# google-research/Splat-SLAM

Hardware: AMD Instinct MI355X
Metric: mapping frames/sec + render ms @640x480, 300k Gaussians; PSNR vs ref (higher is better)
Workload: dtype f32

## Files before the change

splat_slam_amd/csrc/sgr_aux.hip:

```cpp
#include <cmath>

#include <cstdint>

#include "sgr_common.h"

namespace sgr {
int set_error(int code, const char* fmt, ...);


__global__ void __launch_bounds__(256) mapping_loss_kernel(LossTab tab, int HW, float w_rgb, float w_dep, float thr) {
  const int vw = blockIdx.y;
  const float* __restrict__ image = tab.image[vw];
  const float* __restrict__ depth = tab.depth[vw];
  const float* __restrict__ gt_image = tab.gt_image[vw];
  const float* __restrict__ gt_depth = tab.gt_depth[vw];
  float* __restrict__ dimage = tab.dimage[vw];
  float* __restrict__ ddepth = tab.ddepth[vw];
  LossPart* __restrict__ parts = (LossPart*)tab.parts[vw];
  const float ea = tab.exp_a[vw] ? __expf(tab.exp_a[vw][0]) : 1.f;
  const float eb = tab.exp_b[vw] ? tab.exp_b[vw][0] : 0.f;
  LossPart acc = {0.f, 0.f, 0.f, 0.f};
  for (int p = blockIdx.x * blockDim.x + threadIdx.x; p < HW; p += gridDim.x * blockDim.x) {
    float g0 = gt_image[p], g1 = gt_image[HW + p], g2 = gt_image[2 * HW + p];
    bool m = (g0 + g1 + g2) > thr;
// ... 146 lines not shown
                                                       float* __restrict__ s_out, float* __restrict__ r_out,
                                                       float* __restrict__ o_out) {
#pragma clang fp contract(off)
  int64_t i = (int64_t)blockIdx.x * blockDim.x + threadIdx.x;
  if (i >= n) return;
  if (s_out) {
    const F3 sc = ld3(scaling + 3 * i);
    st3(s_out + 3 * i, F3{expf(sc.x), expf(sc.y), expf(sc.z)});
  }
  if (r_out) {
    float4 q = *(const float4*)(rotation + 4 * i);
    float nn = fmaxf(sqrtf(q.x * q.x + q.y * q.y + q.z * q.z + q.w * q.w), 1e-12f);
    *(float4*)(r_out + 4 * i) = make_float4(q.x / nn, q.y / nn, q.z / nn, q.w / nn);
  }
  if (o_out) o_out[i] = 1.f / (1.f + expf(-opacity[i]));
}

#define adam_update(p, g, m, v, GRP, c)                      \
  do {                                                       \
    m = m + (g - m) * (1.f - c.b1);                          \
    v = v * c.b2 + (1.f - c.b2) * g * g;                     \
    float denom_ = sqrtf(v) / c.bc2_sqrt[GRP] + c.eps;       \
    p = p - c.step_size[GRP] * (m / denom_);                 \
  } while (0)

template <int MODE>
__device__ __forceinline__ float take_grad(float* __restrict__ sink, int64_t j, float gathered) {
  if (MODE == 2) return gathered;
  float g = sink[j];
  sink[j] = 0.f;
  return MODE == 1 ? g + gathered : g;
}

template <int MODE>
__device__ __forceinline__ void gaussian_adam_one(int64_t i, const AdamGroups& G, const AdamConst& c, float iso_coef,
                                                  const float* e , float* __restrict__ s_out,
                                                  float* __restrict__ r_out, float* __restrict__ o_out) {
#pragma clang fp contract(off)
#pragma unroll
  for (int grp = 0; grp < 2; ++grp) {
    const SgrAdamGroup& A = G.g[grp];
    if (i < G.r0[grp] || i >= G.r1[grp]) continue;
    float g[3];
    if (MODE == 2) {
      g[0] = e[3 * grp]; g[1] = e[3 * grp + 1]; g[2] = e[3 * grp + 2];
    } else {
      F3 gs = ld3(A.grad + 3 * i);
      st3(A.grad + 3 * i, F3{0.f, 0.f, 0.f});
      g[0] = gs.x; g[1] = gs.y; g[2] = gs.z;
      if (MODE == 1) { g[0] = g[0] + e[3 * grp]; g[1] = g[1] + e[3 * grp + 1]; g[2] = g[2] + e[3 * grp + 2]; }
    }
    if (A.skip) continue;
    F3 p3 = ld3(A.param + 3 * i), m3 = ld3(A.exp_avg + 3 * i), v3 = ld3(A.exp_avg_sq + 3 * i);
    float p[3] = {p3.x, p3.y, p3.z}, m[3] = {m3.x, m3.y, m3.z}, v[3] = {v3.x, v3.y, v3.z};
#pragma unroll
    for (int k = 0; k < 3; ++k) adam_update(p[k], g[k], m[k], v[k], grp, c);
    st3(A.param + 3 * i, F3{p[0], p[1], p[2]});
    st3(A.exp_avg + 3 * i, F3{m[0], m[1], m[2]});
    st3(A.exp_avg_sq + 3 * i, F3{v[0], v[1], v[2]});
  }
  if (i >= G.r0[2] && i < G.r1[2]) {
    const SgrAdamGroup& A = G.g[2];
    float p = A.param[i];
    float sg = 1.f / (1.f + expf(-p));
    float g = take_grad<MODE>(A.grad, i, e[6]) * sg * (1.f - sg);
    if (!A.skip) {
      float m = A.exp_avg[i], v = A.exp_avg_sq[i];
      adam_update(p, g, m, v, 2, c);
      A.param[i] = p; A.exp_avg[i] = m; A.exp_avg_sq[i] = v;
    }
    if (o_out) o_out[i] = 1.f / (1.f + expf(-p));
  }
  if (i >= G.r0[3] && i < G.r1[3]) {
    const SgrAdamGroup& A = G.g[3];
    const F3 p3 = ld3(A.param + 3 * i);
    float p[3] = {p3.x, p3.y, p3.z}, s[3];
#pragma unroll
    for (int k = 0; k < 3; ++k) s[k] = expf(p[k]);
    float mean = (s[0] + s[1] + s[2]) / 3.f;
    float sg[3], ssum = 0.f;
#pragma unroll
    for (int k = 0; k < 3; ++k) { float d = s[k] - mean; sg[k] = d > 0.f ? 1.f : (d < 0.f ? -1.f : 0.f); ssum += sg[k]; }
    float gin[3];
    if (MODE == 2) {
      gin[0] = e[7]; gin[1] = e[8]; gin[2] = e[9];
    } else {
      F3 gs = ld3(A.grad + 3 * i);
      st3(A.grad + 3 * i, F3{0.f, 0.f, 0.f});
      gin[0] = gs.x; gin[1] = gs.y; gin[2] = gs.z;
      if (MODE == 1) { gin[0] = gin[0] + e[7]; gin[1] = gin[1] + e[8]; gin[2] = gin[2] + e[9]; }
    }
    if (!A.skip) {
      F3 m3 = ld3(A.exp_avg + 3 * i), v3 = ld3(A.exp_avg_sq + 3 * i);
      float m[3] = {m3.x, m3.y, m3.z}, v[3] = {v3.x, v3.y, v3.z};
#pragma unroll
      for (int k = 0; k < 3; ++k) {
        float gs = gin[k] + iso_coef * (sg[k] - ssum / 3.f);
        float g = gs * s[k];
        adam_update(p[k], g, m[k], v[k], 3, c);
      }
      st3(A.param + 3 * i, F3{p[0], p[1], p[2]});
      st3(A.exp_avg + 3 * i, F3{m[0], m[1], m[2]});
      st3(A.exp_avg_sq + 3 * i, F3{v[0], v[1], v[2]});
    }
    if (s_out) st3(s_out + 3 * i, F3{expf(p[0]), expf(p[1]), expf(p[2])});
  }
  if (i >= G.r0[4] && i < G.r1[4]) {
    const SgrAdamGroup& A = G.g[4];
    float4 x = *(const float4*)(A.param + 4 * i);
    float4 gy;
    if (MODE == 2) {
      gy = make_float4(e[10], e[11], e[12], e[13]);
    } else {
      gy = *(const float4*)(A.grad + 4 * i);
      *(float4*)(A.grad + 4 * i) = make_float4(0.f, 0.f, 0.f, 0.f);
      if (MODE == 1) { gy.x += e[10]; gy.y += e[11]; gy.z += e[12]; gy.w += e[13]; }
    }
    float nrm = sqrtf(x.x * x.x + x.y * x.y + x.z * x.z + x.w * x.w);
    float gx[4];
    if (nrm > 1e-12f) {
      float inv = 1.f / nrm;
      float y[4] = {x.x * inv, x.y * inv, x.z * inv, x.w * inv};
      float dot = y[0] * gy.x + y[1] * gy.y + y[2] * gy.z + y[3] * gy.w;
      gx[0] = (gy.x - y[0] * dot) * inv; gx[1] = (gy.y - y[1] * dot) * inv;
      gx[2] = (gy.z - y[2] * dot) * inv; gx[3] = (gy.w - y[3] * dot) * inv;
    } else {
      gx[0] = gy.x * 1e12f; gx[1] = gy.y * 1e12f; gx[2] = gy.z * 1e12f; gx[3] = gy.w * 1e12f;
    }
    float pp[4] = {x.x, x.y, x.z, x.w};
    if (!A.skip) {
      float4 m = *(const float4*)(A.exp_avg + 4 * i), v = *(const float4*)(A.exp_avg_sq + 4 * i);
      float mm[4] = {m.x, m.y, m.z, m.w}, vv[4] = {v.x, v.y, v.z, v.w};
#pragma unroll
      for (int k = 0; k < 4; ++k) adam_update(pp[k], gx[k], mm[k], vv[k], 4, c);
      *(float4*)(A.param + 4 * i) = make_float4(pp[0], pp[1], pp[2], pp[3]);
      *(float4*)(A.exp_avg + 4 * i) = make_float4(mm[0], mm[1], mm[2], mm[3]);
      *(float4*)(A.exp_avg_sq + 4 * i) = make_float4(vv[0], vv[1], vv[2], vv[3]);
    }
    if (r_out) {
      float nn = fmaxf(sqrtf(pp[0] * pp[0] + pp[1] * pp[1] + pp[2] * pp[2] + pp[3] * pp[3]), 1e-12f);
      *(float4*)(r_out + 4 * i) = make_float4(pp[0] / nn, pp[1] / nn, pp[2] / nn, pp[3] / nn);
    }
  }
}

__global__ void __launch_bounds__(256) gaussian_adam_kernel(int64_t n, AdamGroups G, AdamConst c, float iso_coef,
                                                            float* __restrict__ s_out, float* __restrict__ r_out,
                                                            float* __restrict__ o_out) {
  int64_t i = (int64_t)blockIdx.x * blockDim.x + threadIdx.x;
  if (i >= n) return;
  const float zero[14] = {0.f, 0.f, 0.f, 0.f, 0.f, 0.f, 0.f, 0.f, 0.f, 0.f, 0.f, 0.f, 0.f, 0.f};
  gaussian_adam_one<0>(i, G, c, iso_coef, zero, s_out, r_out, o_out);
}

template <int MODE>
__global__ void __launch_bounds__(256) gather_adam_kernel(ViewTab tab, int nviews, LOff L, FusedAdam fa) {
  if ((int)blockIdx.x < fa.tail_views) {
    __shared__ LossPart red[4];
    const int v = blockIdx.x;
    loss_final_view((const LossPart*)fa.tail_parts[v], fa.tail_nparts, fa.tail_inv_rgb, fa.tail_inv_dep, fa.tail_alpha,
                    fa.tail_loss[v], fa.tail_da[v], fa.tail_db[v], red);
    if (threadIdx.x == 0 && fa.exp_rows > 0 && fa.tail_da[v] && ((const SavedHeader*)tab.saved[v])->overflow == 0u) {
      const ptrdiff_t d = fa.tail_da[v] - fa.exp_grad;
      if (d >= 0 && d < (ptrdiff_t)fa.exp_rows * fa.exp_width && d % fa.exp_width == 0) {
        const int r = (int)(d / fa.exp_width);
        if (fa.exp_active[r])
          masked_adam_row(r, fa.exp_width, fa.exp_param, fa.exp_grad, fa.exp_avg, fa.exp_avg_sq, fa.exp_step, fa.exp_lr,
                          fa.exp_b1, fa.exp_b2, fa.exp_eps);
      }
    }
    return;
  }
  __shared__ const char* s_scratch[kMaxViews];
  __shared__ const int32_t* s_radii[kMaxViews];
  __shared__ uint32_t s_over[kMaxViews];
#pragma unroll
  for (int u = 0; u < kMaxViews; ++u)
    if ((int)threadIdx.x == u && u < nviews) {
      s_scratch[u] = tab.scratch[u];
      s_radii[u] = tab.radii[u];
      s_over[u] = ((const SavedHeader*)tab.saved[u])->overflow;
    }
  __syncthreads();
  uint32_t truncated = 0u;
  for (int u = 0; u < nviews; ++u) truncated |= (s_over[u] != 0u ? 1u : 0u) << u;
  const int i = ((int)blockIdx.x - fa.tail_views) * blockDim.x + threadIdx.x;
  if (i >= L.N) return;
  float a[14];
#pragma unroll
  for (int k = 0; k < 14; ++k) a[k] = 0.f;
  float st_norm = 0.f, st_cnt = 0.f, st_maxr = 0.f;
  uint32_t seen = 0u;
  for (int p = 0; p < min(L.k1_parts, nviews); ++p) seen |= ((const uint32_t*)(tab.saved[0] + L.o_vismask))[(size_t)p * L.N + i];
  seen &= ~truncated;
  const bool any = seen != 0u;
  while (seen) {
    const int v = __builtin_ctz(seen);
    seen &= seen - 1u;
    const float4* rec = (const float4*)(s_scratch[v] + L.o_gradrec) + (size_t)i * 4;
    const int r = s_radii[v][i];
    float4 r0 = rec[0], r1 = rec[1], r2 = rec[2], r3 = rec[3];
    a[0] += r0.x; a[1] += r0.y; a[2] += r0.z; a[3] += r0.w; a[4] += r1.x; a[5] += r1.y; a[6] += r1.z; a[7] += r1.w;
    a[8] += r2.x; a[9] += r2.y; a[10] += r2.z; a[11] += r2.w; a[12] += r3.x; a[13] += r3.y;
    st_norm += sqrtf(r3.z * r3.z + r3.w * r3.w);
    st_cnt += 1.f;
    st_maxr = fmaxf(st_maxr, (float)r);
  }
  if (any && fa.stat_accum) {
    fa.stat_accum[i] += st_norm;
    fa.stat_denom[i] += st_cnt;
    fa.stat_maxr[i] = fmaxf(fa.stat_maxr[i], st_maxr);
  }
  if (MODE == 3) {
    if (!any) return;
    float* g0 = fa.G.g[0].grad + 3 * (size_t)i; float* g1 = fa.G.g[1].grad + 3 * (size_t)i; float* g3 = fa.G.g[3].grad + 3 * (size_t)i;
    float* g4 = fa.G.g[4].grad + 4 * (size_t)i;
    g0[0] += a[0]; g0[1] += a[1]; g0[2] += a[2];
    g1[0] += a[3]; g1[1] += a[4]; g1[2] += a[5];
    fa.G.g[2].grad[i] += a[6];
    g3[0] += a[7]; g3[1] += a[8]; g3[2] += a[9];
    g4[0] += a[10]; g4[1] += a[11]; g4[2] += a[12]; g4[3] += a[13];
    return;
  }
  if (MODE == 4) {
    st3(fa.G.g[0].grad + 3 * (size_t)i, F3{a[0], a[1], a[2]});
    st3(fa.G.g[1].grad + 3 * (size_t)i, F3{a[3], a[4], a[5]});
    fa.G.g[2].grad[i] = a[6];
    st3(fa.G.g[3].grad + 3 * (size_t)i, F3{a[7], a[8], a[9]});
    *(float4*)(fa.G.g[4].grad + 4 * (size_t)i) = make_float4(a[10], a[11], a[12], a[13]);
    return;
  }
  gaussian_adam_one<MODE >= 3 ? 1 : MODE>(i, fa.G, fa.c, fa.iso_coef, a, fa.s_out, fa.r_out, fa.o_out);
}

// ... 523 lines not shown
```

splat_slam_amd/csrc/sgr_common.h:

```cpp
#pragma once

#include <hip/hip_runtime.h>
#include <stdint.h>

#include "../../include/splat_hip.h"

namespace sgr {

constexpr float kNearPlane = 0.001f;
constexpr float kAlphaMin = 1.0f / 255.0f;
constexpr float kAlphaMax = 0.99f;
constexpr float kTEps = 1e-4f;
constexpr float kDilation = 0.3f;
constexpr float kTouchedT = 0.5f;
constexpr int kRefTile = 16;
constexpr int kTile = 8;
constexpr int kWave = 64;
constexpr int kCntSlotWords = 8;
constexpr uint32_t kTileCountLimit = 0xff00u;
__host__ __device__ inline size_t tile_counter_word(int x, int y, int gxp) { return ((size_t)(y >> 1) * gxp + (x >> 1)) * (kCntSlotWords / 2); }
__host__ __device__ inline int tile_counter_shift(int x, int y) { return 16 * ((y & 1) * 2 + (x & 1)); }
constexpr int kK1MaxParts = 4;
#ifndef SGR_K1_DENSE_PARTS
#define SGR_K1_DENSE_PARTS 2
// ... 72 lines not shown
  uint32_t max_rendered;
  uint32_t counts_read;
  uint32_t pad;
};
static_assert(sizeof(SavedHeader) == 64, "the header is one 64-byte record (sgr_query_header copies 16 words)");

inline __host__ __device__ size_t align_up(size_t x, size_t a = 256) { return (x + a - 1) / a * a; }

constexpr int kMaxViews = 16;
struct ViewTab {
  const float* viewmatrix[kMaxViews];
  const float* projmatrix[kMaxViews];
  const float* campos[kMaxViews];
  const float* projraw[kMaxViews];
  char* saved[kMaxViews];
  char* scratch[kMaxViews];
  float* color[kMaxViews];
  float* depth[kMaxViews];
  float* opacity[kMaxViews];
  int32_t* radii[kMaxViews];
  int32_t* n_touched[kMaxViews];
  const float* dL_dcolor[kMaxViews];
  const float* dL_ddepth[kMaxViews];
  float* dL_dtau[kMaxViews];
  float* dL_dmeans2D[kMaxViews];
};
struct LOff {
  int N, H, W, gx, gy, gxp, sgx, sgy, ntiles, pre_blocks, nseg, dbg, mean_hint, k1_parts;
  uint32_t sgx_magic;
  __host__ void set_hint(int h) { mean_hint = h; k1_parts = k1_parts_for(nseg, h); }
  int64_t cap;
  size_t o_hdr, o_tile_count, o_grec, o_point_list, o_ranges,
      o_tile_maxc, o_final_T, o_tile_order, o_block_touched, o_block_vis, o_block_base_t, o_block_base_v, o_vis_list,
      o_seg_list, o_vismask, o_entries, o_bucket, o_ovf, o_partials, o_tau_part, o_gradrec, o_taurec;
};
#ifndef SGR_TILE_ORDER_MIN_LIST
#define SGR_TILE_ORDER_MIN_LIST 64
#endif
__host__ __device__ inline bool tile_order_used(const LOff& L) { return !(L.mean_hint != 0 && L.mean_hint <= SGR_TILE_ORDER_MIN_LIST); }
struct __attribute__((aligned(16))) OvfEntry { uint32_t tile, rank; uint64_t key; };
struct Common {
  int deg, M;
  int upstream_pose_jac;
  float tanfovx, tanfovy, mod;
  const float* bg;
};

int debug_flags();

struct __attribute__((aligned(16))) GRec {
  float px, py;
  uint32_t rect01, rect23;
  float A, B, C, opacity;
  float r, g, b, depth;
  uint32_t touched, offset, vis_pos, clamped;
};
static_assert(sizeof(GRec) == 64, "GRec must be one 64-byte record");
struct Rect { int x0, y0, x1, y1; };
__device__ __forceinline__ Rect unpack_rect(uint32_t r01, uint32_t r23) {
  return {(int)(r01 & 0xffffu), (int)(r01 >> 16), (int)(r23 & 0xffffu), (int)(r23 >> 16)};
}

struct Layout {
  int N, H, W;
  int64_t cap;
  int gx, gy, ntiles;
  int sgx, sgy;
  int tile_bits;
  size_t o_hdr, o_tile_count, o_grec, o_point_list, o_ranges,
      o_tile_maxc, o_final_T, o_tile_order, o_block_touched, o_block_vis, o_block_base_t, o_block_base_v, o_vis_list,
      o_seg_list, o_vismask, saved_bytes, zero_bytes;
  size_t o_entries, o_bucket, o_ovf;
  size_t o_partials, o_tau_part, o_gradrec, o_taurec, scratch_bytes;
  int pre_blocks, nseg;

  __host__ Layout(int N_, int H_, int W_, int64_t cap_) : N(N_), H(H_), W(W_), cap(cap_) {
    gx = (W + kTile - 1) / kTile;
    gy = (H + kTile - 1) / kTile;
    ntiles = gx * gy;
    sgx = (W + kRefTile - 1) / kRefTile;
    sgy = (H + kRefTile - 1) / kRefTile;
    tile_bits = 1;
    while ((1ll << tile_bits) < (long long)ntiles + 1) ++tile_bits;
    size_t o = 0;
    auto take = [&](size_t bytes) { size_t r = o; o = align_up(o + bytes); return r; };
    size_t n = (size_t)(N > 0 ? N : 1), c = (size_t)(cap > 0 ? cap : 1);
    pre_blocks = (N + 255) / 256;
    nseg = (N + kSeg - 1) / kSeg;
    size_t nb = (size_t)(pre_blocks > 0 ? pre_blocks : 1);
    o_hdr = take(sizeof(SavedHeader));
    o_tile_count = take((size_t)((gy + 1) / 2) * ((gx + 1) / 2) * 4 * kCntSlotWords);
    zero_bytes = o;
    o_grec = take(n * sizeof(GRec));
    o_point_list = take(c * 4);
    o_ranges = take((size_t)ntiles * 8 * kRngStride);
    o_tile_maxc = take((size_t)ntiles * 4);
    o_final_T = take((size_t)ntiles * 64 * 8);
    o_tile_order = take((size_t)sgx * sgy * 4 + 16);
    o_block_touched = take(nb * 4);
    o_block_vis = take(nb * 4);
    o_block_base_t = take(nb * 4);
    o_block_base_v = take(nb * 4);
    o_vis_list = take(n * 4);
    o_seg_list = take(n * 4);
    o_vismask = take(n * 4 * kK1MaxParts);
    saved_bytes = o;

    o = 0;
    o_entries = take(c * 8);
    o_bucket = take((size_t)ntiles * kBucket * 8);
    o_ovf = take(c * sizeof(OvfEntry));
    o_partials = take(c * 48);
    o_tau_part = take((size_t)(pre_blocks > 0 ? pre_blocks : 1) * 6 * 4);
    o_gradrec = take(n * 64);
    o_taurec = take(n * 24);
    scratch_bytes = o;
  }
  __host__ LOff dev() const {
    LOff d;
    d.N = N; d.H = H; d.W = W; d.gx = gx; d.gy = gy; d.gxp = (gx + 1) / 2; d.sgx = sgx; d.sgy = sgy; d.ntiles = ntiles; d.pre_blocks = pre_blocks; d.nseg = nseg; d.dbg = debug_flags(); d.mean_hint = 0; d.k1_parts = k1_parts_for(nseg); d.sgx_magic = (uint32_t)((1ull << 32) / (uint64_t)(sgx > 0 ? sgx : 1)) + 1u;
    d.cap = cap;
    d.o_hdr = o_hdr; d.o_tile_count = o_tile_count; d.o_grec = o_grec;
    d.o_point_list = o_point_list; d.o_ranges = o_ranges; d.o_tile_maxc = o_tile_maxc; d.o_final_T = o_final_T;
    d.o_tile_order = o_tile_order; d.o_block_touched = o_block_touched; d.o_block_vis = o_block_vis;
    d.o_block_base_t = o_block_base_t; d.o_block_base_v = o_block_base_v; d.o_vis_list = o_vis_list;
    d.o_seg_list = o_seg_list; d.o_vismask = o_vismask; d.o_entries = o_entries; d.o_bucket = o_bucket; d.o_ovf = o_ovf; d.o_partials = o_partials; d.o_tau_part = o_tau_part;
    d.o_gradrec = o_gradrec; d.o_taurec = o_taurec;
    return d;
  }
};

struct LossTab {
  const float* image[kMaxViews];
  const float* depth[kMaxViews];
  const float* gt_image[kMaxViews];
  const float* gt_depth[kMaxViews];
  const float* exp_a[kMaxViews];
  const float* exp_b[kMaxViews];
  float* loss[kMaxViews];
  float* dimage[kMaxViews];
  float* ddepth[kMaxViews];
  float* da[kMaxViews];
  float* db[kMaxViews];
  void* parts[kMaxViews];
};
void launch_mapping_loss(const LossTab& tab, int nviews, int HW, float alpha, float thr, float upstream, hipStream_t st);
void launch_mapping_loss_final(const LossTab& tab, int nviews, int HW, int nparts, float alpha, hipStream_t st);
struct LossPart { float rgb, dep, da, db; };
size_t ssim_term_view_maps(int H, int W);
int ssim_loss_nparts(int H, int W);
void launch_ssim_mapping_loss(const LossTab& lt, int v0, int nv, int H, int W, float alpha, float lam, float thr, float upstream,
                              float* maps, hipStream_t st);
struct LossCoef { float w_rgb, w_dep, thr; };

struct AdamConst { float b1, b2, eps; float bc2_sqrt[5], step_size[5]; };
struct AdamGroups { SgrAdamGroup g[5]; int64_t r0[5], r1[5]; };
struct FusedAdam {
  AdamGroups G;
  AdamConst c;
  float iso_coef;
// ... 4 lines not shown
  int tail_views, tail_nparts;
  float tail_inv_rgb, tail_inv_dep, tail_alpha;
  const void* tail_parts[kMaxViews];
  float* tail_loss[kMaxViews];
  float* tail_da[kMaxViews];
  float* tail_db[kMaxViews];
  int exp_rows, exp_width;
  float* exp_param; const float* exp_grad; float* exp_avg; float* exp_avg_sq; int32_t* exp_step; const int32_t* exp_active;
  float exp_lr, exp_b1, exp_b2, exp_eps;
};
int make_fused_adam(int64_t n, const SgrAdamGroup groups[5], float beta1, float beta2, float eps, float iso_weight, FusedAdam* out);
int gaussian_adam_step_act(int64_t n, const SgrAdamGroup groups[5], float beta1, float beta2, float eps, float iso_weight,
                           float* s_out, float* r_out, float* o_out, void* stream);
void launch_gather_adam(const ViewTab& tab, int nviews, const LOff& L, const FusedAdam& fa, hipStream_t st);

enum ProfKind { PK_PRE_FWD = 0, PK_SCAN, PK_SCATTER, PK_BLEND_FUSED, PK_BLEND_FWD, PK_BLEND_BWD, PK_PRE_BWD };
void prof_begin(int kind, hipStream_t st);
void prof_end(int kind, hipStream_t st);
struct ProfScope {
  int kind; hipStream_t st;
  ProfScope(int k, hipStream_t s) : kind(k), st(s) { prof_begin(kind, st); }
  ~ProfScope() { prof_end(kind, st); }
};

__device__ __forceinline__ uint32_t abs_offset(const char* saved, const LOff& L, uint32_t g, uint32_t rel_offset) {
  return rel_offset + ((const uint32_t*)(saved + L.o_block_base_t))[g >> kSegShift];
}
__device__ __forceinline__ const GRec* grec_of(const char* saved, const LOff& L) { return (const GRec*)(saved + L.o_grec); }

struct __attribute__((packed, aligned(4))) F3 { float x, y, z; };
__device__ __forceinline__ F3 ld3(const float* p) { return *(const F3*)p; }
__device__ __forceinline__ void st3(float* p, F3 v) { *(F3*)p = v; }

struct V3 { float x, y, z; };
__device__ __forceinline__ V3 cross(V3 a, V3 b) {
  return {a.y * b.z - a.z * b.y, a.z * b.x - a.x * b.z, a.x * b.y - a.y * b.x};
}

template <int CTRL, int ROW_MASK = 0xf, int BANK_MASK = 0xf>
__device__ __forceinline__ float dpp_f(float old, float v) {
  return __builtin_bit_cast(float, __builtin_amdgcn_update_dpp(__builtin_bit_cast(int, old),
                                                                __builtin_bit_cast(int, v), CTRL, ROW_MASK,
                                                                BANK_MASK, false));
}
constexpr int DPP_ROW_SHR1 = 0x111, DPP_ROW_SHR2 = 0x112, DPP_ROW_SHR4 = 0x114, DPP_ROW_SHR8 = 0x118;
constexpr int DPP_WAVE_SHR1 = 0x138, DPP_ROW_BCAST15 = 0x142, DPP_ROW_BCAST31 = 0x143;

__device__ __forceinline__ float wave_scan_add(float v) {
  v += dpp_f<DPP_ROW_SHR1>(0.f, v);
  v += dpp_f<DPP_ROW_SHR2>(0.f, v);
  v += dpp_f<DPP_ROW_SHR4>(0.f, v);
  v += dpp_f<DPP_ROW_SHR8>(0.f, v);
  v += dpp_f<DPP_ROW_BCAST15, 0xa>(0.f, v);
  v += dpp_f<DPP_ROW_BCAST31, 0xc>(0.f, v);
  return v;
}
__device__ __forceinline__ float wave_scan_mul(float v) {
  v *= dpp_f<DPP_ROW_SHR1>(1.f, v);
  v *= dpp_f<DPP_ROW_SHR2>(1.f, v);
  v *= dpp_f<DPP_ROW_SHR4>(1.f, v);
  v *= dpp_f<DPP_ROW_SHR8>(1.f, v);
  v *= dpp_f<DPP_ROW_BCAST15, 0xa>(1.f, v);
  v *= dpp_f<DPP_ROW_BCAST31, 0xc>(1.f, v);
  return v;
}
template <int CTRL, int ROW_MASK = 0xf>
// ... 41 lines not shown
```

splat_slam_amd/csrc/sgr_preprocess.hip:

```cpp
#include "sgr_common.h"

namespace sgr {

struct Cam {
  float vm[16];
  float pm[16];
};

__device__ __forceinline__ void load16(const float* __restrict__ src, float* dst) {
#pragma unroll
  for (int i = 0; i < 16; ++i) dst[i] = src[i];
}

__device__ __forceinline__ void quat_to_R(const float q[4], float R[3][3]) {
  float r = q[0], x = q[1], y = q[2], z = q[3];
  R[0][0] = 1.f - 2.f * (y * y + z * z); R[0][1] = 2.f * (x * y - r * z); R[0][2] = 2.f * (x * z + r * y);
  R[1][0] = 2.f * (x * y + r * z); R[1][1] = 1.f - 2.f * (x * x + z * z); R[1][2] = 2.f * (y * z - r * x);
  R[2][0] = 2.f * (x * z - r * y); R[2][1] = 2.f * (y * z + r * x); R[2][2] = 1.f - 2.f * (x * x + y * y);
}

__device__ __forceinline__ void cov3d_from_scale_rot(const float s[3], float mod, const float q[4], float S6[6]) {
  float R[3][3];
  quat_to_R(q, R);
  float M[3][3];
// ... 814 lines not shown
      float r = q[0], x = q[1], y = q[2], z = q[3];
      g_q[0] = 2.f * (-z * dR[0][1] + y * dR[0][2] + z * dR[1][0] - x * dR[1][2] - y * dR[2][0] + x * dR[2][1]);
      g_q[1] = 2.f * (y * dR[0][1] + z * dR[0][2] + y * dR[1][0] - 2.f * x * dR[1][1] - r * dR[1][2] + z * dR[2][0] + r * dR[2][1] - 2.f * x * dR[2][2]);
      g_q[2] = 2.f * (-2.f * y * dR[0][0] + x * dR[0][1] + r * dR[0][2] + x * dR[1][0] + z * dR[1][2] - r * dR[2][0] + z * dR[2][1] - 2.f * y * dR[2][2]);
      g_q[3] = 2.f * (-2.f * z * dR[0][0] - r * dR[0][1] + x * dR[0][2] + r * dR[1][0] - 2.f * z * dR[1][1] + y * dR[1][2] + x * dR[2][0] + y * dR[2][1]);
    }
  }
  (void)dcolors;
#pragma unroll
  for (int k = 0; k < 3; ++k) { acc.p[k] += g_p[k]; acc.s[k] += g_s[k]; acc.rgb_or_sh0[k] += sh0[k]; }
#pragma unroll
  for (int k = 0; k < 4; ++k) acc.q[k] += g_q[k];
#pragma unroll
  for (int k = 0; k < 6; ++k) acc.S6[k] += g_S6[k];
  acc.op += g_op;
  acc.m2[0] = g_m2[0]; acc.m2[1] = g_m2[1];
}

template <int LPG>
__global__ void __launch_bounds__(256) __attribute__((amdgpu_waves_per_eu(3, 8))) preprocess_bwd_dense_kernel(
    ViewTab tab, LOff L, Common cm, const float* __restrict__ means3D, const float* __restrict__ shs,
    const float* __restrict__ colors_precomp, const float* __restrict__ scales, const float* __restrict__ rotations,
    const float* __restrict__ cov3D_precomp, float* __restrict__ dshs, float* __restrict__ dcov3D, int accumulate) {
  const int v = blockIdx.y;
  const char* saved = tab.saved[v];
  const int V = (int)((const SavedHeader*)(saved + L.o_hdr))->num_visible;
  constexpr int kPerBlock = 256 / LPG;
  if ((int)(blockIdx.x * kPerBlock) >= V) return;
  const int t = blockIdx.x * kPerBlock + (int)threadIdx.x / LPG;
  const bool have = t < V;
  const int i = have ? (int)((const uint32_t*)(saved + L.o_vis_list))[t] : 0;
  uint4 q3 = make_uint4(0u, 0u, 0u, 0u);
  float4 g0 = make_float4(0.f, 0.f, 0.f, 0.f), g1 = g0;
  if (have) {
    const float4* rec = (const float4*)(grec_of(saved, L) + i);
    g0 = rec[0]; g1 = rec[1]; q3 = ((const uint4*)rec)[3];
  }
  const uint32_t my_r01 = __float_as_uint(g0.z), my_r23 = __float_as_uint(g0.w);
  const bool tested = have && footprint_worthwhile((int)(my_r23 & 0xffffu) - (int)(my_r01 & 0xffffu), (int)(my_r23 >> 16) - (int)(my_r01 >> 16));
  const Footprint foot = tested ? make_footprint(g0.x, g0.y, g1.x, g1.y, g1.z, g1.w, 0.006f)
                                : Footprint{0.f, 0.f, 0.f, 0.f, 0.f, 0.f, 0.f, -1.f};
  auto slot_unwritten = [](const Footprint& f, uint32_t r01, uint32_t r23, uint32_t k) -> bool {
    if (!(f.thr >= 0.f)) return false;
    const int x0 = (int)(r01 & 0xffffu), y0 = (int)(r01 >> 16), w = (int)(r23 & 0xffffu) - x0;
    int q = (int)(((float)k + 0.5f) * __builtin_amdgcn_rcpf((float)w));
    int rem = (int)k - q * w;
    if (rem < 0) { --q; rem += w; }
    if (rem >= w) { ++q; rem -= w; }
    return footprint_qmin(f, x0 + rem, y0 + q) > f.thr;
  };
  constexpr uint32_t kLongRun = 96u;
  float gsum[10];
  {
    const float4* __restrict__ partials = (const float4*)(tab.scratch[v] + L.o_partials);
    const int lane = threadIdx.x & 63, grp = lane >> 3, sub = lane & 7;
    const uint32_t my_off = have ? abs_offset(saved, L, (uint32_t)i, q3.y) : 0u, my_cnt = have ? q3.x : 0u;
#pragma unroll
    for (int j = 0; j < 10; ++j) gsum[j] = 0.f;
    const int longest = __builtin_amdgcn_readfirstlane(wave_max_i32((int)my_cnt));
    constexpr uint32_t kLongRunQuad = 192u;
    if constexpr (LPG == 4) {
      const uint32_t q = (uint32_t)lane & 3u;
      const uint32_t c = my_cnt > kLongRunQuad ? 0u : my_cnt;
      for (uint32_t k0 = q; k0 < c; k0 += 12u) {
        float4 ld[9];
#pragma unroll
        for (int u = 0; u < 3; ++u) {
          const uint32_t k = k0 + 4u * (uint32_t)u;
          const uint64_t e = (uint64_t)my_off + k;
          const bool in = k < c && (int64_t)e < L.cap && !slot_unwritten(foot, my_r01, my_r23, k);
#pragma unroll
          for (int w = 0; w < 3; ++w) ld[3 * u + w] = in ? partials[e * 3 + w] : make_float4(0.f, 0.f, 0.f, 0.f);
        }
#pragma unroll
        for (int u = 0; u < 3; ++u) {
          const float4 p0 = ld[3 * u], p1 = ld[3 * u + 1], p2 = ld[3 * u + 2];
          gsum[0] += p0.x; gsum[1] += p0.y; gsum[2] += p0.z; gsum[3] += p0.w; gsum[4] += p1.x;
          gsum[5] += p1.y; gsum[6] += p1.z; gsum[7] += p1.w; gsum[8] += p2.x; gsum[9] += p2.y;
        }
      }
#pragma unroll
      for (int off = 1; off < 4; off <<= 1)
#pragma unroll
        for (int j = 0; j < 10; ++j) gsum[j] += __shfl_xor(gsum[j], off);
    } else if (longest <= 6) {
      for (uint32_t k0 = 0; k0 < my_cnt; k0 += 3u) {
        float4 ld[9];
#pragma unroll
        for (int u = 0; u < 3; ++u) {
          const uint64_t e = (uint64_t)my_off + k0 + (uint32_t)u;
          const bool in = k0 + (uint32_t)u < my_cnt && (int64_t)e < L.cap && !slot_unwritten(foot, my_r01, my_r23, k0 + (uint32_t)u);
#pragma unroll
          for (int w = 0; w < 3; ++w) ld[3 * u + w] = in ? partials[e * 3 + w] : make_float4(0.f, 0.f, 0.f, 0.f);
        }
#pragma unroll
        for (int u = 0; u < 3; ++u) {
          const float4 p0 = ld[3 * u], p1 = ld[3 * u + 1], p2 = ld[3 * u + 2];
          gsum[0] += p0.x; gsum[1] += p0.y; gsum[2] += p0.z; gsum[3] += p0.w; gsum[4] += p1.x;
          gsum[5] += p1.y; gsum[6] += p1.z; gsum[7] += p1.w; gsum[8] += p2.x; gsum[9] += p2.y;
        }
      }
    } else
#pragma unroll 1
    for (int r = 0; r < (LPG == 1 ? 8 : 0); ++r) {
      const int src = r * 8 + grp;
      const uint32_t o = (uint32_t)__shfl((int)my_off, src), c_all = (uint32_t)__shfl((int)my_cnt, src);
      const uint32_t c = c_all > kLongRun ? 0u : c_all;
      const uint32_t s01 = (uint32_t)__shfl((int)my_r01, src), s23 = (uint32_t)__shfl((int)my_r23, src);
      const Footprint sf{__shfl(foot.px, src), __shfl(foot.py, src), __shfl(foot.A, src), __shfl(foot.B, src),
                         __shfl(foot.C, src), __shfl(foot.invA, src), __shfl(foot.invC, src), __shfl(foot.thr, src)};
      float part[10];
#pragma unroll
      for (int j = 0; j < 10; ++j) part[j] = 0.f;
      for (uint32_t k0 = (uint32_t)sub; k0 < c; k0 += 24u) {
        float4 ld[9];
#pragma unroll
        for (int u = 0; u < 3; ++u) {
          const uint32_t k = k0 + 8u * (uint32_t)u;
          const uint64_t e = (uint64_t)o + k;
          const bool in = k < c && (int64_t)e < L.cap && !slot_unwritten(sf, s01, s23, k);
#pragma unroll
          for (int w = 0; w < 3; ++w) ld[3 * u + w] = in ? partials[e * 3 + w] : make_float4(0.f, 0.f, 0.f, 0.f);
        }
#pragma unroll
        for (int u = 0; u < 3; ++u) {
          const float4 p0 = ld[3 * u], p1 = ld[3 * u + 1], p2 = ld[3 * u + 2];
          part[0] += p0.x; part[1] += p0.y; part[2] += p0.z; part[3] += p0.w; part[4] += p1.x;
          part[5] += p1.y; part[6] += p1.z; part[7] += p1.w; part[8] += p2.x; part[9] += p2.y;
        }
      }
#pragma unroll
      for (int off = 1; off < 8; off <<= 1)
#pragma unroll
        for (int j = 0; j < 10; ++j) part[j] += __shfl_xor(part[j], off);
#pragma unroll
      for (int j = 0; j < 10; ++j) {
        const float got = __shfl(part[j], sub * 8);
        if (grp == r) gsum[j] = got;
      }
    }
    constexpr uint32_t kWholeWave = LPG == 4 ? kLongRunQuad : kLongRun;
    if (longest > (int)kWholeWave) {
      unsigned long long lm = __ballot(my_cnt > kWholeWave && (LPG == 1 || (lane & (LPG - 1)) == 0));
      while (lm != 0ull) {
        const int src = __builtin_amdgcn_readfirstlane(__ffsll((long long)lm) - 1);
        lm &= lm - 1ull;
        const uint32_t o = (uint32_t)__shfl((int)my_off, src), c = (uint32_t)__shfl((int)my_cnt, src);
        const uint32_t s01 = (uint32_t)__shfl((int)my_r01, src), s23 = (uint32_t)__shfl((int)my_r23, src);
        const Footprint sf{__shfl(foot.px, src), __shfl(foot.py, src), __shfl(foot.A, src), __shfl(foot.B, src),
                           __shfl(foot.C, src), __shfl(foot.invA, src), __shfl(foot.invC, src), __shfl(foot.thr, src)};
        float part[10];
#pragma unroll
        for (int j = 0; j < 10; ++j) part[j] = 0.f;
        for (uint32_t k0 = (uint32_t)lane; k0 < c; k0 += 192u) {
          float4 ld[9];
#pragma unroll
          for (int u = 0; u < 3; ++u) {
            const uint32_t k = k0 + 64u * (uint32_t)u;
            const uint64_t e = (uint64_t)o + k;
            const bool in = k < c && (int64_t)e < L.cap && !slot_unwritten(sf, s01, s23, k);
#pragma unroll
            for (int w = 0; w < 3; ++w) ld[3 * u + w] = in ? partials[e * 3 + w] : make_float4(0.f, 0.f, 0.f, 0.f);
          }
#pragma unroll
          for (int u = 0; u < 3; ++u) {
            const float4 p0 = ld[3 * u], p1 = ld[3 * u + 1], p2 = ld[3 * u + 2];
            part[0] += p0.x; part[1] += p0.y; part[2] += p0.z; part[3] += p0.w; part[4] += p1.x;
            part[5] += p1.y; part[6] += p1.z; part[7] += p1.w; part[8] += p2.x; part[9] += p2.y;
          }
        }
#pragma unroll
        for (int off = 1; off < 64; off <<= 1)
#pragma unroll
          for (int j = 0; j < 10; ++j) part[j] += __shfl_xor(part[j], off);
        if ((lane & ~(LPG - 1)) == src)
#pragma unroll
          for (int j = 0; j < 10; ++j) gsum[j] = part[j];
      }
    }
  }
  if (!have || (LPG > 1 && (threadIdx.x & (LPG - 1)) != 0)) return;
  {
    const float G0 = gsum[0], G1 = gsum[1], Gxx = gsum[2], Gxy = gsum[3], Go = gsum[4], Gr = gsum[5], Gg = gsum[6], Gb = gsum[7],
                Gyy = gsum[8], Gd = gsum[9];
    gsum[0] = (-(g1.x * G0) - g1.y * G1) * (0.5f * (float)L.W);
    gsum[1] = (-(g1.z * G1) - g1.y * G0) * (0.5f * (float)L.H);
    gsum[2] = -0.5f * Gxx;
    gsum[3] = -Gxy;
    gsum[4] = -0.5f * Gyy;
    gsum[5] = Go; gsum[6] = Gr; gsum[7] = Gg; gsum[8] = Gb; gsum[9] = Gd;
  }
  float tau[6] = {0.f, 0.f, 0.f, 0.f, 0.f, 0.f};
  GaussGrad acc;
#pragma unroll
  for (int j = 0; j < 3; ++j) { acc.p[j] = 0.f; acc.s[j] = 0.f; acc.rgb_or_sh0[j] = 0.f; }
#pragma unroll
  for (int j = 0; j < 4; ++j) acc.q[j] = 0.f;
#pragma unroll
  for (int j = 0; j < 6; ++j) acc.S6[j] = 0.f;
  acc.op = 0.f; acc.m2[0] = 0.f; acc.m2[1] = 0.f;
  preprocess_bwd_one_view(i, L.H, L.W, cm.deg, cm.M, cm.tanfovx, cm.tanfovy, cm.mod, tab.viewmatrix[v], tab.projmatrix[v],
                          tab.projraw[v], tab.campos[v], means3D, shs, colors_precomp, scales, rotations, cov3D_precomp,
                          gsum, q3.w, dshs, accumulate, acc, tau, cm.upstream_pose_jac);
  float4* rec = (float4*)(tab.scratch[v] + L.o_gradrec) + (size_t)i * 4;
  rec[0] = make_float4(acc.p[0], acc.p[1], acc.p[2], acc.rgb_or_sh0[0]);
  rec[1] = make_float4(acc.rgb_or_sh0[1], acc.rgb_or_sh0[2], acc.op, acc.s[0]);
  rec[2] = make_float4(acc.s[1], acc.s[2], acc.q[0], acc.q[1]);
  rec[3] = make_float4(acc.q[2], acc.q[3], acc.m2[0], acc.m2[1]);
  if (float* m2 = tab.dL_dmeans2D[v]) {
    if (((const SavedHeader*)(saved + L.o_hdr))->overflow == 0u) {
      m2[3 * (size_t)i] = acc.m2[0];
      m2[3 * (size_t)i + 1] = acc.m2[1];
    }
  }
  if (dcov3D) {
#pragma unroll
    for (int j = 0; j < 6; ++j) { if (accumulate) dcov3D[6 * i + j] += acc.S6[j]; else dcov3D[6 * i + j] = acc.S6[j]; }
  }
  if (tab.dL_dtau[v]) {
    float* tr = (float*)(tab.scratch[v] + L.o_taurec) + (size_t)t * 6;
#pragma unroll
    for (int j = 0; j < 6; ++j) tr[j] = tau[j];
  }
}

__global__ void __launch_bounds__(256) grad_gather_kernel(
    ViewTab tab, int nviews, LOff L, int deg, int M, int has_colors, float* __restrict__ dmeans3D,
    float* __restrict__ dmeans2D, float* __restrict__ dopac, float* __restrict__ dshs, float* __restrict__ dcolors,
    float* __restrict__ dscales, float* __restrict__ drots, float* __restrict__ dcov3D, int accumulate,
    float* __restrict__ stat_accum, float* __restrict__ stat_denom, float* __restrict__ stat_maxr) {
  __shared__ float red[4][6];
  const int i = blockIdx.x * blockDim.x + threadIdx.x;
  const bool in_range = i < L.N;
  float a[14];
#pragma unroll
  for (int k = 0; k < 14; ++k) a[k] = 0.f;
  float m2x = 0.f, m2y = 0.f, st_norm = 0.f, st_cnt = 0.f, st_maxr = 0.f;
  bool any = false;
  for (int v = 0; v < nviews; ++v) {
    const bool truncated = ((const SavedHeader*)tab.saved[v])->overflow != 0u;
    const int r = in_range && !truncated ? tab.radii[v][i] : 0;
    uint32_t pos = 0;
    if (r > 0) {
      any = true;
      if (tab.dL_dtau[v]) pos = grec_of(tab.saved[v], L)[i].vis_pos;
      const float4* rec = (const float4*)(tab.scratch[v] + L.o_gradrec) + (size_t)i * 4;
      float4 r0 = rec[0], r1 = rec[1], r2 = rec[2], r3 = rec[3];
      a[0] += r0.x; a[1] += r0.y; a[2] += r0.z; a[3] += r0.w; a[4] += r1.x; a[5] += r1.y; a[6] += r1.z; a[7] += r1.w;
      a[8] += r2.x; a[9] += r2.y; a[10] += r2.z; a[11] += r2.w; a[12] += r3.x; a[13] += r3.y;
      m2x += r3.z; m2y += r3.w;
      st_norm += sqrtf(r3.z * r3.z + r3.w * r3.w);
      st_cnt += 1.f;
      st_maxr = fmaxf(st_maxr, (float)r);
    }
    if (tab.dL_dtau[v]) {
      const float* tr = (const float*)(tab.scratch[v] + L.o_taurec) + (size_t)pos * 6;
      int lane = threadIdx.x & 63, wv = threadIdx.x >> 6;
#pragma unroll
      for (int k = 0; k < 6; ++k) {
        float s = wave_sum(r > 0 ? tr[k] : 0.f);
        if (lane == 0) red[wv][k] = s;
      }
      __syncthreads();
      if (threadIdx.x < 6) {
        int k = threadIdx.x;
        ((float*)(tab.scratch[v] + L.o_tau_part))[(size_t)blockIdx.x * 6 + k] = ((red[0][k] + red[1][k]) + red[2][k]) + red[3][k];
      }
      __syncthreads();
    }
  }
  if (!in_range) return;
  float* sh0 = has_colors ? dcolors : dshs;
  const size_t sh_stride = has_colors ? 3 : (size_t)M * 3;
  if (accumulate) {
    if (!any) return;
    if (dmeans3D) { dmeans3D[3 * i] += a[0]; dmeans3D[3 * i + 1] += a[1]; dmeans3D[3 * i + 2] += a[2]; }
    if (sh0 && (has_colors || deg == 0)) { sh0[i * sh_stride] += a[3]; sh0[i * sh_stride + 1] += a[4]; sh0[i * sh_stride + 2] += a[5]; }
    if (dopac) dopac[i] += a[6];
    if (dscales) { dscales[3 * i] += a[7]; dscales[3 * i + 1] += a[8]; dscales[3 * i + 2] += a[9]; }
// ... 80 lines not shown
```

Before: 61.72.

## Compact per-view gradient records by visible rank and use nontemporal streaming accesses

```diff
diff --git a/splat_slam_amd/csrc/sgr_aux.hip b/splat_slam_amd/csrc/sgr_aux.hip
--- a/splat_slam_amd/csrc/sgr_aux.hip
+++ b/splat_slam_amd/csrc/sgr_aux.hip
@@ -202,6 +202,13 @@
   return MODE == 1 ? g + gathered : g;
 }
 
+#ifndef SGR_STREAM_ACT
+#define SGR_STREAM_ACT 0
+#endif
+__device__ __forceinline__ void act_st1(float* p, float v) { if (SGR_STREAM_ACT) st1_stream(p, v); else *p = v; }
+__device__ __forceinline__ void act_st3(float* p, F3 v) { if (SGR_STREAM_ACT) st3_stream(p, v); else st3(p, v); }
+__device__ __forceinline__ void act_st4(float* p, float4 v) { if (SGR_STREAM_ACT) st4_stream(p, v); else *(float4*)p = v; }
+
 template <int MODE>
 __device__ __forceinline__ void gaussian_adam_one(int64_t i, const AdamGroups& G, const AdamConst& c, float iso_coef,
                                                   const float* e , float* __restrict__ s_out,
@@ -221,29 +228,29 @@
       if (MODE == 1) { g[0] = g[0] + e[3 * grp]; g[1] = g[1] + e[3 * grp + 1]; g[2] = g[2] + e[3 * grp + 2]; }
     }
     if (A.skip) continue;
-    F3 p3 = ld3(A.param + 3 * i), m3 = ld3(A.exp_avg + 3 * i), v3 = ld3(A.exp_avg_sq + 3 * i);
+    F3 p3 = ld3_stream(A.param + 3 * i), m3 = ld3_stream(A.exp_avg + 3 * i), v3 = ld3_stream(A.exp_avg_sq + 3 * i);
     float p[3] = {p3.x, p3.y, p3.z}, m[3] = {m3.x, m3.y, m3.z}, v[3] = {v3.x, v3.y, v3.z};
 #pragma unroll
     for (int k = 0; k < 3; ++k) adam_update(p[k], g[k], m[k], v[k], grp, c);
-    st3(A.param + 3 * i, F3{p[0], p[1], p[2]});
-    st3(A.exp_avg + 3 * i, F3{m[0], m[1], m[2]});
-    st3(A.exp_avg_sq + 3 * i, F3{v[0], v[1], v[2]});
+    st3_stream(A.param + 3 * i, F3{p[0], p[1], p[2]});
+    st3_stream(A.exp_avg + 3 * i, F3{m[0], m[1], m[2]});
+    st3_stream(A.exp_avg_sq + 3 * i, F3{v[0], v[1], v[2]});
   }
   if (i >= G.r0[2] && i < G.r1[2]) {
     const SgrAdamGroup& A = G.g[2];
-    float p = A.param[i];
+    float p = ld1_stream(A.param + i);
     float sg = 1.f / (1.f + expf(-p));
     float g = take_grad<MODE>(A.grad, i, e[6]) * sg * (1.f - sg);
     if (!A.skip) {
-      float m = A.exp_avg[i], v = A.exp_avg_sq[i];
+      float m = ld1_stream(A.exp_avg + i), v = ld1_stream(A.exp_avg_sq + i);
       adam_update(p, g, m, v, 2, c);
-      A.param[i] = p; A.exp_avg[i] = m; A.exp_avg_sq[i] = v;
-    }
-    if (o_out) o_out[i] = 1.f / (1.f + expf(-p));
+      st1_stream(A.param + i, p); st1_stream(A.exp_avg + i, m); st1_stream(A.exp_avg_sq + i, v);
+    }
+    if (o_out) act_st1(o_out + i, 1.f / (1.f + expf(-p)));
   }
   if (i >= G.r0[3] && i < G.r1[3]) {
     const SgrAdamGroup& A = G.g[3];
-    const F3 p3 = ld3(A.param + 3 * i);
+    const F3 p3 = ld3_stream(A.param + 3 * i);
     float p[3] = {p3.x, p3.y, p3.z}, s[3];
 #pragma unroll
     for (int k = 0; k < 3; ++k) s[k] = expf(p[k]);
@@ -261,7 +268,7 @@
       if (MODE == 1) { gin[0] = gin[0] + e[7]; gin[1] = gin[1] + e[8]; gin[2] = gin[2] + e[9]; }
     }
     if (!A.skip) {
-      F3 m3 = ld3(A.exp_avg + 3 * i), v3 = ld3(A.exp_avg_sq + 3 * i);
+      F3 m3 = ld3_stream(A.exp_avg + 3 * i), v3 = ld3_stream(A.exp_avg_sq + 3 * i);
       float m[3] = {m3.x, m3.y, m3.z}, v[3] = {v3.x, v3.y, v3.z};
 #pragma unroll
       for (int k = 0; k < 3; ++k) {
@@ -269,15 +276,15 @@
         float g = gs * s[k];
         adam_update(p[k], g, m[k], v[k], 3, c);
       }
-      st3(A.param + 3 * i, F3{p[0], p[1], p[2]});
-      st3(A.exp_avg + 3 * i, F3{m[0], m[1], m[2]});
-      st3(A.exp_avg_sq + 3 * i, F3{v[0], v[1], v[2]});
-    }
-    if (s_out) st3(s_out + 3 * i, F3{expf(p[0]), expf(p[1]), expf(p[2])});
+      st3_stream(A.param + 3 * i, F3{p[0], p[1], p[2]});
+      st3_stream(A.exp_avg + 3 * i, F3{m[0], m[1], m[2]});
+      st3_stream(A.exp_avg_sq + 3 * i, F3{v[0], v[1], v[2]});
+    }
+    if (s_out) act_st3(s_out + 3 * i, F3{expf(p[0]), expf(p[1]), expf(p[2])});
   }
   if (i >= G.r0[4] && i < G.r1[4]) {
     const SgrAdamGroup& A = G.g[4];
-    float4 x = *(const float4*)(A.param + 4 * i);
+    float4 x = ld4_stream(A.param + 4 * i);
     float4 gy;
     if (MODE == 2) {
       gy = make_float4(e[10], e[11], e[12], e[13]);
@@ -299,17 +306,17 @@
     }
     float pp[4] = {x.x, x.y, x.z, x.w};
     if (!A.skip) {
-      float4 m = *(const float4*)(A.exp_avg + 4 * i), v = *(const float4*)(A.exp_avg_sq + 4 * i);
+      float4 m = ld4_stream(A.exp_avg + 4 * i), v = ld4_stream(A.exp_avg_sq + 4 * i);
       float mm[4] = {m.x, m.y, m.z, m.w}, vv[4] = {v.x, v.y, v.z, v.w};
 #pragma unroll
       for (int k = 0; k < 4; ++k) adam_update(pp[k], gx[k], mm[k], vv[k], 4, c);
-      *(float4*)(A.param + 4 * i) = make_float4(pp[0], pp[1], pp[2], pp[3]);
-      *(float4*)(A.exp_avg + 4 * i) = make_float4(mm[0], mm[1], mm[2], mm[3]);
-      *(float4*)(A.exp_avg_sq + 4 * i) = make_float4(vv[0], vv[1], vv[2], vv[3]);
+      st4_stream(A.param + 4 * i, make_float4(pp[0], pp[1], pp[2], pp[3]));
+      st4_stream(A.exp_avg + 4 * i, make_float4(mm[0], mm[1], mm[2], mm[3]));
+      st4_stream(A.exp_avg_sq + 4 * i, make_float4(vv[0], vv[1], vv[2], vv[3]));
     }
     if (r_out) {
       float nn = fmaxf(sqrtf(pp[0] * pp[0] + pp[1] * pp[1] + pp[2] * pp[2] + pp[3] * pp[3]), 1e-12f);
-      *(float4*)(r_out + 4 * i) = make_float4(pp[0] / nn, pp[1] / nn, pp[2] / nn, pp[3] / nn);
+      act_st4(r_out + 4 * i, make_float4(pp[0] / nn, pp[1] / nn, pp[2] / nn, pp[3] / nn));
     }
   }
 }
@@ -342,34 +349,56 @@
     return;
   }
   __shared__ const char* s_scratch[kMaxViews];
-  __shared__ const int32_t* s_radii[kMaxViews];
   __shared__ uint32_t s_over[kMaxViews];
+  __shared__ uint32_t s_base[kMaxViews];
+  __shared__ __attribute__((aligned(16))) uint32_t s_wcnt[kMaxViews][4];
+  const int blk = (int)blockIdx.x - fa.tail_views;
 #pragma unroll
   for (int u = 0; u < kMaxViews; ++u)
     if ((int)threadIdx.x == u && u < nviews) {
       s_scratch[u] = tab.scratch[u];
-      s_radii[u] = tab.radii[u];
       s_over[u] = ((const SavedHeader*)tab.saved[u])->overflow;
+      s_base[u] = ((const uint32_t*)(tab.saved[u] + L.o_block_base_v))[blk];
     }
   __syncthreads();
   uint32_t truncated = 0u;
   for (int u = 0; u < nviews; ++u) truncated |= (s_over[u] != 0u ? 1u : 0u) << u;
-  const int i = ((int)blockIdx.x - fa.tail_views) * blockDim.x + threadIdx.x;
-  if (i >= L.N) return;
+  const int i = blk * (int)blockDim.x + (int)threadIdx.x;
   float a[14];
 #pragma unroll
   for (int k = 0; k < 14; ++k) a[k] = 0.f;
   float st_norm = 0.f, st_cnt = 0.f, st_maxr = 0.f;
   uint32_t seen = 0u;
-  for (int p = 0; p < min(L.k1_parts, nviews); ++p) seen |= ((const uint32_t*)(tab.saved[0] + L.o_vismask))[(size_t)p * L.N + i];
+  if (i < L.N)
+    for (int p = 0; p < min(L.k1_parts, nviews); ++p) seen |= ((const uint32_t*)(tab.saved[0] + L.o_vismask))[(size_t)p * L.N + i];
+  uint32_t wrank[kMaxViews / 4];
+#pragma unroll
+  for (int k = 0; k < kMaxViews / 4; ++k) wrank[k] = 0u;
+  {
+    const int lane = threadIdx.x & 63, wv = threadIdx.x >> 6;
+#pragma unroll
+    for (int u = 0; u < kMaxViews; ++u) {
+      if (u < nviews) {
+        const unsigned long long m = __ballot((seen >> u) & 1u);
+        wrank[u >> 2] |= (uint32_t)__popcll(m & ((1ull << lane) - 1ull)) << ((u & 3) * 8);
+        if (lane == 0) s_wcnt[u][wv] = (uint32_t)__popcll(m);
+      }
+    }
+  }
+  __syncthreads();
+  if (i >= L.N) return;
   seen &= ~truncated;
   const bool any = seen != 0u;
   while (seen) {
     const int v = __builtin_ctz(seen);
     seen &= seen - 1u;
-    const float4* rec = (const float4*)(s_scratch[v] + L.o_gradrec) + (size_t)i * 4;
-    const int r = s_radii[v][i];
-    float4 r0 = rec[0], r1 = rec[1], r2 = rec[2], r3 = rec[3];
+    const int wv = threadIdx.x >> 6;
+    const uint4 wc = *(const uint4*)s_wcnt[v];
+    const uint32_t rank = min(s_base[v] + (wv > 0 ? wc.x : 0u) + (wv > 1 ? wc.y : 0u) + (wv > 2 ? wc.z : 0u) + ((wrank[v >> 2] >> ((v & 3) * 8)) & 0xffu),
+                              (uint32_t)(L.N - 1));
+    const float* rec = (const float*)(s_scratch[v] + L.o_gradrec) + (size_t)rank * 16;
+    const int r = __float_as_int(ld1_stream((const float*)(s_scratch[v] + L.o_radrec) + rank));
+    float4 r0 = ld4_stream(rec), r1 = ld4_stream(rec + 4), r2 = ld4_stream(rec + 8), r3 = ld4_stream(rec + 12);
     a[0] += r0.x; a[1] += r0.y; a[2] += r0.z; a[3] += r0.w; a[4] += r1.x; a[5] += r1.y; a[6] += r1.z; a[7] += r1.w;
     a[8] += r2.x; a[9] += r2.y; a[10] += r2.z; a[11] += r2.w; a[12] += r3.x; a[13] += r3.y;
     st_norm += sqrtf(r3.z * r3.z + r3.w * r3.w);
diff --git a/splat_slam_amd/csrc/sgr_common.h b/splat_slam_amd/csrc/sgr_common.h
--- a/splat_slam_amd/csrc/sgr_common.h
+++ b/splat_slam_amd/csrc/sgr_common.h
@@ -128,7 +128,7 @@
   int64_t cap;
   size_t o_hdr, o_tile_count, o_grec, o_point_list, o_ranges,
       o_tile_maxc, o_final_T, o_tile_order, o_block_touched, o_block_vis, o_block_base_t, o_block_base_v, o_vis_list,
-      o_seg_list, o_vismask, o_entries, o_bucket, o_ovf, o_partials, o_tau_part, o_gradrec, o_taurec;
+      o_seg_list, o_vismask, o_entries, o_bucket, o_ovf, o_partials, o_tau_part, o_gradrec, o_taurec, o_radrec;
 };
 #ifndef SGR_TILE_ORDER_MIN_LIST
 #define SGR_TILE_ORDER_MIN_LIST 64
@@ -167,7 +167,7 @@
       o_tile_maxc, o_final_T, o_tile_order, o_block_touched, o_block_vis, o_block_base_t, o_block_base_v, o_vis_list,
       o_seg_list, o_vismask, saved_bytes, zero_bytes;
   size_t o_entries, o_bucket, o_ovf;
-  size_t o_partials, o_tau_part, o_gradrec, o_taurec, scratch_bytes;
+  size_t o_partials, o_tau_part, o_gradrec, o_taurec, o_radrec, scratch_bytes;
   int pre_blocks, nseg;
 
   __host__ Layout(int N_, int H_, int W_, int64_t cap_) : N(N_), H(H_), W(W_), cap(cap_) {
@@ -210,6 +210,7 @@
     o_tau_part = take((size_t)(pre_blocks > 0 ? pre_blocks : 1) * 6 * 4);
     o_gradrec = take(n * 64);
     o_taurec = take(n * 24);
+    o_radrec = take(n * 4);
     scratch_bytes = o;
   }
   __host__ LOff dev() const {
@@ -221,7 +222,7 @@
     d.o_tile_order = o_tile_order; d.o_block_touched = o_block_touched; d.o_block_vis = o_block_vis;
     d.o_block_base_t = o_block_base_t; d.o_block_base_v = o_block_base_v; d.o_vis_list = o_vis_list;
     d.o_seg_list = o_seg_list; d.o_vismask = o_vismask; d.o_entries = o_entries; d.o_bucket = o_bucket; d.o_ovf = o_ovf; d.o_partials = o_partials; d.o_tau_part = o_tau_part;
-    d.o_gradrec = o_gradrec; d.o_taurec = o_taurec;
+    d.o_gradrec = o_gradrec; d.o_taurec = o_taurec; d.o_radrec = o_radrec;
     return d;
   }
 };
@@ -292,6 +293,54 @@
 __device__ __forceinline__ F3 ld3(const float* p) { return *(const F3*)p; }
 __device__ __forceinline__ void st3(float* p, F3 v) { *(F3*)p = v; }
 
+#ifndef SGR_STREAM_NT
+#define SGR_STREAM_NT 1
+#endif
+typedef float v4f_t __attribute__((ext_vector_type(4)));
+__device__ __forceinline__ float ld1_stream(const float* p) {
+#if SGR_STREAM_NT
+  return __builtin_nontemporal_load(p);
+#else
+  return *p;
+#endif
+}
+__device__ __forceinline__ void st1_stream(float* p, float v) {
+#if SGR_STREAM_NT
+  __builtin_nontemporal_store(v, p);
+#else
+  *p = v;
+#endif
+}
+__device__ __forceinline__ F3 ld3_stream(const float* p) {
+#if SGR_STREAM_NT
+  return F3{__builtin_nontemporal_load(p), __builtin_nontemporal_load(p + 1), __builtin_nontemporal_load(p + 2)};
+#else
+  return ld3(p);
+#endif
+}
+__device__ __forceinline__ void st3_stream(float* p, F3 v) {
+#if SGR_STREAM_NT
+  __builtin_nontemporal_store(v.x, p); __builtin_nontemporal_store(v.y, p + 1); __builtin_nontemporal_store(v.z, p + 2);
+#else
+  st3(p, v);
+#endif
+}
+__device__ __forceinline__ float4 ld4_stream(const float* p) {
+#if SGR_STREAM_NT
+  const v4f_t v = __builtin_nontemporal_load((const v4f_t*)p);
+  return make_float4(v.x, v.y, v.z, v.w);
+#else
+  return *(const float4*)p;
+#endif
+}
+__device__ __forceinline__ void st4_stream(float* p, float4 v) {
+#if SGR_STREAM_NT
+  __builtin_nontemporal_store(v4f_t{v.x, v.y, v.z, v.w}, (v4f_t*)p);
+#else
+  *(float4*)p = v;
+#endif
+}
+
 struct V3 { float x, y, z; };
 __device__ __forceinline__ V3 cross(V3 a, V3 b) {
   return {a.y * b.z - a.z * b.y, a.z * b.x - a.x * b.z, a.x * b.y - a.y * b.x};
diff --git a/splat_slam_amd/csrc/sgr_preprocess.hip b/splat_slam_amd/csrc/sgr_preprocess.hip
--- a/splat_slam_amd/csrc/sgr_preprocess.hip
+++ b/splat_slam_amd/csrc/sgr_preprocess.hip
@@ -870,9 +870,11 @@
   const int i = have ? (int)((const uint32_t*)(saved + L.o_vis_list))[t] : 0;
   uint4 q3 = make_uint4(0u, 0u, 0u, 0u);
   float4 g0 = make_float4(0.f, 0.f, 0.f, 0.f), g1 = g0;
+  int my_radius = 0;
   if (have) {
     const float4* rec = (const float4*)(grec_of(saved, L) + i);
     g0 = rec[0]; g1 = rec[1]; q3 = ((const uint4*)rec)[3];
+    my_radius = tab.radii[v][i];
   }
   const uint32_t my_r01 = __float_as_uint(g0.z), my_r23 = __float_as_uint(g0.w);
   const bool tested = have && footprint_worthwhile((int)(my_r23 & 0xffffu) - (int)(my_r01 & 0xffffu), (int)(my_r23 >> 16) - (int)(my_r01 >> 16));
@@ -908,7 +910,7 @@
           const uint64_t e = (uint64_t)my_off + k;
           const bool in = k < c && (int64_t)e < L.cap && !slot_unwritten(foot, my_r01, my_r23, k);
 #pragma unroll
-          for (int w = 0; w < 3; ++w) ld[3 * u + w] = in ? partials[e * 3 + w] : make_float4(0.f, 0.f, 0.f, 0.f);
+          for (int w = 0; w < 3; ++w) ld[3 * u + w] = in ? ld4_stream((const float*)(partials + (e * 3 + w))) : make_float4(0.f, 0.f, 0.f, 0.f);
         }
 #pragma unroll
         for (int u = 0; u < 3; ++u) {
@@ -929,7 +931,7 @@
           const uint64_t e = (uint64_t)my_off + k0 + (uint32_t)u;
           const bool in = k0 + (uint32_t)u < my_cnt && (int64_t)e < L.cap && !slot_unwritten(foot, my_r01, my_r23, k0 + (uint32_t)u);
 #pragma unroll
-          for (int w = 0; w < 3; ++w) ld[3 * u + w] = in ? partials[e * 3 + w] : make_float4(0.f, 0.f, 0.f, 0.f);
+          for (int w = 0; w < 3; ++w) ld[3 * u + w] = in ? ld4_stream((const float*)(partials + (e * 3 + w))) : make_float4(0.f, 0.f, 0.f, 0.f);
         }
 #pragma unroll
         for (int u = 0; u < 3; ++u) {
@@ -958,7 +960,7 @@
           const uint64_t e = (uint64_t)o + k;
           const bool in = k < c && (int64_t)e < L.cap && !slot_unwritten(sf, s01, s23, k);
 #pragma unroll
-          for (int w = 0; w < 3; ++w) ld[3 * u + w] = in ? partials[e * 3 + w] : make_float4(0.f, 0.f, 0.f, 0.f);
+          for (int w = 0; w < 3; ++w) ld[3 * u + w] = in ? ld4_stream((const float*)(partials + (e * 3 + w))) : make_float4(0.f, 0.f, 0.f, 0.f);
         }
 #pragma unroll
         for (int u = 0; u < 3; ++u) {
@@ -998,7 +1000,7 @@
             const uint64_t e = (uint64_t)o + k;
             const bool in = k < c && (int64_t)e < L.cap && !slot_unwritten(sf, s01, s23, k);
 #pragma unroll
-            for (int w = 0; w < 3; ++w) ld[3 * u + w] = in ? partials[e * 3 + w] : make_float4(0.f, 0.f, 0.f, 0.f);
+            for (int w = 0; w < 3; ++w) ld[3 * u + w] = in ? ld4_stream((const float*)(partials + (e * 3 + w))) : make_float4(0.f, 0.f, 0.f, 0.f);
           }
 #pragma unroll
           for (int u = 0; u < 3; ++u) {
@@ -1040,11 +1042,12 @@
   preprocess_bwd_one_view(i, L.H, L.W, cm.deg, cm.M, cm.tanfovx, cm.tanfovy, cm.mod, tab.viewmatrix[v], tab.projmatrix[v],
                           tab.projraw[v], tab.campos[v], means3D, shs, colors_precomp, scales, rotations, cov3D_precomp,
                           gsum, q3.w, dshs, accumulate, acc, tau, cm.upstream_pose_jac);
-  float4* rec = (float4*)(tab.scratch[v] + L.o_gradrec) + (size_t)i * 4;
-  rec[0] = make_float4(acc.p[0], acc.p[1], acc.p[2], acc.rgb_or_sh0[0]);
-  rec[1] = make_float4(acc.rgb_or_sh0[1], acc.rgb_or_sh0[2], acc.op, acc.s[0]);
-  rec[2] = make_float4(acc.s[1], acc.s[2], acc.q[0], acc.q[1]);
-  rec[3] = make_float4(acc.q[2], acc.q[3], acc.m2[0], acc.m2[1]);
+  float* rec = (float*)(tab.scratch[v] + L.o_gradrec) + (size_t)t * 16;
+  st4_stream(rec, make_float4(acc.p[0], acc.p[1], acc.p[2], acc.rgb_or_sh0[0]));
+  st4_stream(rec + 4, make_float4(acc.rgb_or_sh0[1], acc.rgb_or_sh0[2], acc.op, acc.s[0]));
+  st4_stream(rec + 8, make_float4(acc.s[1], acc.s[2], acc.q[0], acc.q[1]));
+  st4_stream(rec + 12, make_float4(acc.q[2], acc.q[3], acc.m2[0], acc.m2[1]));
+  ((int32_t*)(tab.scratch[v] + L.o_radrec))[t] = my_radius;
   if (float* m2 = tab.dL_dmeans2D[v]) {
     if (((const SavedHeader*)(saved + L.o_hdr))->overflow == 0u) {
       m2[3 * (size_t)i] = acc.m2[0];
@@ -1081,8 +1084,8 @@
     uint32_t pos = 0;
     if (r > 0) {
       any = true;
-      if (tab.dL_dtau[v]) pos = grec_of(tab.saved[v], L)[i].vis_pos;
-      const float4* rec = (const float4*)(tab.scratch[v] + L.o_gradrec) + (size_t)i * 4;
+      pos = min(grec_of(tab.saved[v], L)[i].vis_pos, (uint32_t)(L.N - 1));
+      const float4* rec = (const float4*)(tab.scratch[v] + L.o_gradrec) + (size_t)pos * 4;
       float4 r0 = rec[0], r1 = rec[1], r2 = rec[2], r3 = rec[3];
       a[0] += r0.x; a[1] += r0.y; a[2] += r0.z; a[3] += r0.w; a[4] += r1.x; a[5] += r1.y; a[6] += r1.z; a[7] += r1.w;
       a[8] += r2.x; a[9] += r2.y; a[10] += r2.z; a[11] += r2.w; a[12] += r3.x; a[13] += r3.y;
```

Result: slower. 58.41 (-5.4%).
